# fujii-team/deComP

Measured on AMD Instinct MI355X. Metric: nmf_mu_iterations_per_s, higher is better.
Workload: dtype f32

## Files before the change

### decomp_amd/csrc/gemm.hpp

```cpp
#pragma once
#include <type_traits>

#include "gemm_generic.hpp"
#include "gemm_mfma_bf16x6.hpp"
#include "gemm_mfma_f32.hpp"
#include "gemm_mfma_f64.hpp"
#include "scalar.hpp"

namespace dcp {

enum GemmForm { FORM_NT = 0, FORM_NN = 1, FORM_TN = 2 };
enum TileSel { TILE_AUTO = 0, TILE_LARGE = 1, TILE_SMALL = 2, TILE_HUGE = 3, TILE_SMALL_DEEP = 4, TILE_MID = 5 };

template <class T>
struct GemmArgs {
    const T* A = nullptr;
    long lda = 0;
    const T* B = nullptr;
    long ldb = 0;
    const T* B2 = nullptr;
    long ldb2 = 0;
    int n_b1 = 0;
    const T* A2 = nullptr;
    long lda2 = 0;
// ... 316 lines not shown
    } else {
        if constexpr (std::is_same<T, c64>::value) {
            if (cplx_on_mfma<FORM>(a.conjA, a.conjB, a.ext_ws)) {
                GemmProblem p;
                const float* Ar = reinterpret_cast<const float*>(a.A);
                p.A = Ar; p.lda = 2 * a.lda;
                p.B2 = nullptr; p.ldb2 = 0; p.n_b1 = 2 * a.N;
                p.ksplits = a.ksplits; p.klen = a.klen;
                p.tiles_m = p.tiles_n = 0;
                p.mt_fast = (FORM == FORM_NT) ? 0 : 1;
                constexpr int AL = (FORM == FORM_TN) ? XMAJOR : KMAJOR;
                constexpr int BL = (FORM == FORM_NT) ? KMAJOR : XMAJOR;
                if constexpr (FORM == FORM_TN) {
                    p.B = reinterpret_cast<const float*>(a.B); p.ldb = 2 * a.ldb;
                    if (a.B2 != nullptr) {
                        p.B2 = reinterpret_cast<const float*>(a.B2); p.ldb2 = 2 * a.ldb2;
                        p.n_b1 = 2 * a.n_b1;
                    }
                    p.M = 2 * a.M; p.N = 2 * a.N; p.K = a.K;
                    CplxTnEpi<Epi> ce{epi};
                    const int tier = pick_tier<FORM>(p.M, p.N, p.K, a.tile, a.split_planned);
                    if (tier == TIER_SMALL || tier == TIER_SMALL_DEEP || tier == TIER_FLAT || tier == TIER_TALL)
                        return launch_gemm_mfma<CfgSmall, AL, BL>(stream, p, ce);
                    if (!tn_plain_schedule()) return launch_gemm_mfma<CfgLargeX, AL, BL>(stream, p, ce);
                    return launch_gemm_mfma<CfgLarge, AL, BL>(stream, p, ce);
                } else if (cplx_planar_a<FORM>(a.M, a.N, a.conjA, a.conjB, a.ext_ws)) {
                    if (a.A_rows != nullptr) {
                        p.A = a.A_rows; p.lda = a.lda_rows;
                    } else {
                        long g = ((long)a.M * a.K + 255) / 256;
                        if (g > 4096) g = 4096;
                        if (g < 1) g = 1;
                        hipLaunchKernelGGL((cplx_rows_kernel<float>), dim3((unsigned)g), dim3(256), 0, stream, a.A,
                                           (long)a.M, (long)a.K, a.lda, a.ext_ws);
                        p.A = a.ext_ws; p.lda = a.K;
                    }
                    p.B = reinterpret_cast<const float*>(a.B); p.ldb = 2 * a.ldb;
                    p.M = 2 * a.M; p.N = 2 * a.N; p.K = a.K;
                    if (a.ksplits <= 1) p.klen = 0;
                    CplxNnEpi<Epi> ce{epi};
                    const int tier = pick_tier<FORM>(p.M, p.N, p.K, a.tile, a.split_planned);
                    if (tier == TIER_SMALL_DEEP) return launch_gemm_mfma<CfgSmallDeep, AL, BL>(stream, p, ce);
                    if (tier == TIER_SMALL || tier == TIER_FLAT || tier == TIER_TALL)
                        return launch_gemm_mfma<CfgSmall, AL, BL>(stream, p, ce);
                    return launch_gemm_mfma<CfgLarge, AL, BL>(stream, p, ce);
                } else {
                    const long rowsB = (FORM == FORM_NT) ? a.N : a.K;
                    const long colsB = (FORM == FORM_NT) ? a.K : a.N;
                    long g = (rowsB * colsB + 255) / 256;
                    if (g > 4096) g = 4096;
                    if (g < 1) g = 1;
                    if (!a.ext_ready)
                        hipLaunchKernelGGL((cplx_ext_kernel<float>), dim3((unsigned)g), dim3(256), 0, stream, a.B,
                                           rowsB, colsB, a.ldb, a.ext_ws);
                    p.B = a.ext_ws; p.ldb = 2 * colsB;
                    p.M = a.M; p.N = 2 * a.N; p.K = 2 * a.K;
                    if (a.ksplits <= 1) p.klen = 0;
                    CplxColEpi<Epi> ce{epi};
                    const int tier = pick_tier<FORM>(p.M, p.N, p.K, a.tile, a.split_planned);
                    if (tier == TIER_SMALL || tier == TIER_SMALL_DEEP || tier == TIER_FLAT || tier == TIER_TALL)
                        return launch_gemm_mfma<CfgSmall, AL, BL>(stream, p, ce);
                    if (tier == TIER_HUGE) return launch_gemm_mfma<CfgHuge, AL, BL>(stream, p, ce);
                    if (tier == TIER_MID) return launch_gemm_mfma<CfgMid, AL, BL>(stream, p, ce);
                    return launch_gemm_mfma<CfgLarge, AL, BL>(stream, p, ce);
                }
            }
        }
        if constexpr (std::is_same<T, c128>::value) {
            const int Me = (FORM == FORM_TN) ? 2 * a.M : a.M;
            const int t128 = f64_tier(Me, 2 * a.N, a.tile);
            if (cplx_on_mfma<FORM>(a.conjA, a.conjB, a.ext_ws) && t128 != F64_GENERIC) {
                GemmProblemD p;
                p.A = reinterpret_cast<const double*>(a.A); p.lda = 2 * a.lda;
                p.B2 = nullptr; p.ldb2 = 0; p.n_b1 = 2 * a.N;
                p.ksplits = a.ksplits; p.klen = a.klen;
                p.tiles_m = p.tiles_n = 0;
                p.mt_fast = (FORM == FORM_NT) ? 0 : 1;
                constexpr int AL = (FORM == FORM_TN) ? XMAJOR : KMAJOR;
                constexpr int BL = (FORM == FORM_NT) ? KMAJOR : XMAJOR;
                if constexpr (FORM == FORM_TN) {
                    p.B = reinterpret_cast<const double*>(a.B); p.ldb = 2 * a.ldb;
                    if (a.B2 != nullptr) {
                        p.B2 = reinterpret_cast<const double*>(a.B2); p.ldb2 = 2 * a.ldb2;
                        p.n_b1 = 2 * a.n_b1;
                    }
                    p.M = 2 * a.M; p.N = 2 * a.N; p.K = a.K;
                    CplxTnEpi<Epi, double> ce{epi};
                    return launch_f64_tier<AL, BL>(t128, stream, p, ce);
                } else if (cplx_planar_a<FORM>(a.M, a.N, a.conjA, a.conjB, a.ext_ws) &&
                           f64_tier(2 * a.M, 2 * a.N, a.tile) != F64_GENERIC) {
                    if (a.A_rows != nullptr) {
                        p.A = a.A_rows; p.lda = a.lda_rows;
                    } else {
                        long g = ((long)a.M * a.K + 255) / 256;
                        if (g > 4096) g = 4096;
                        if (g < 1) g = 1;
                        hipLaunchKernelGGL((cplx_rows_kernel<double>), dim3((unsigned)g), dim3(256), 0, stream, a.A,
                                           (long)a.M, (long)a.K, a.lda, a.ext_ws);
                        p.A = a.ext_ws; p.lda = a.K;
                    }
                    p.B = reinterpret_cast<const double*>(a.B); p.ldb = 2 * a.ldb;
                    p.M = 2 * a.M; p.N = 2 * a.N; p.K = a.K;
                    if (a.ksplits <= 1) p.klen = 0;
                    CplxNnEpi<Epi, double> ce{epi};
                    return launch_f64_tier<AL, BL>(f64_tier(p.M, p.N, a.tile), stream, p, ce);
                } else {
                    const long rowsB = (FORM == FORM_NT) ? a.N : a.K;
                    const long colsB = (FORM == FORM_NT) ? a.K : a.N;
                    long g = (rowsB * colsB + 255) / 256;
                    if (g > 4096) g = 4096;
                    if (g < 1) g = 1;
                    if (!a.ext_ready)
                        hipLaunchKernelGGL((cplx_ext_kernel<double>), dim3((unsigned)g), dim3(256), 0, stream, a.B,
                                           rowsB, colsB, a.ldb, a.ext_ws);
                    p.B = a.ext_ws; p.ldb = 2 * colsB;
                    p.M = a.M; p.N = 2 * a.N; p.K = 2 * a.K;
                    if (a.ksplits <= 1) p.klen = 0;
                    CplxColEpi<Epi, double> ce{epi};
                    return launch_f64_tier<AL, BL>(t128, stream, p, ce);
                }
            }
        }
        if constexpr (std::is_same<T, double>::value) {
            const int t64 = f64_tier(a.M, a.N, a.tile, a.K);
            if (t64 != F64_GENERIC) {
                GemmProblemD p;
                p.A = a.A; p.lda = a.lda; p.B = a.B; p.ldb = a.ldb;
                p.B2 = a.B2; p.ldb2 = a.ldb2; p.n_b1 = a.n_b1;
                p.M = a.M; p.N = a.N; p.K = a.K;
                p.ksplits = a.ksplits; p.klen = a.klen;
                p.tiles_m = p.tiles_n = 0;
                p.mt_fast = (FORM == FORM_NT) ? 0 : 1;
                constexpr int AL = (FORM == FORM_TN) ? XMAJOR : KMAJOR;
                constexpr int BL = (FORM == FORM_NT) ? KMAJOR : XMAJOR;
                return launch_f64_tier<AL, BL>(t64, stream, p, epi);
            }
        }
        GenericProblem<T> p;
        p.A = a.A; p.B = a.B; p.B2 = a.B2; p.n_b1 = a.n_b1;
        if (FORM == FORM_TN) { p.sAm = 1; p.sAk = a.lda; } else { p.sAm = a.lda; p.sAk = 1; }
        if (FORM == FORM_NT) { p.sBk = 1; p.sBn = a.ldb; p.sB2k = 1; p.sB2n = a.ldb2; }
        else { p.sBk = a.ldb; p.sBn = 1; p.sB2k = a.ldb2; p.sB2n = 1; }
        p.M = a.M; p.N = a.N; p.K = a.K;
        p.ksplits = a.ksplits; p.klen = a.klen;
        p.tiles_m = p.tiles_n = 0;
        if constexpr (scalar_traits<T>::is_complex)
            return launch_gemm_generic<T, Epi>(stream, p, a.conjA, a.conjB, epi);
        else
            return launch_gemm_generic<T, Epi>(stream, p, false, false, epi);
    }
}

enum { X6_NONE = -1, X6_LARGE = 0, X6_HUGE = 1 };

template <int FORM>
inline GemmProblem x6_problem(const GemmArgs<float>& a) {
    GemmProblem p;
    p.A = a.A; p.lda = a.lda; p.B = a.B; p.ldb = a.ldb;
    p.B2 = a.B2; p.ldb2 = a.ldb2; p.n_b1 = a.n_b1;
    p.A2 = a.A2; p.lda2 = a.lda2; p.m_a1 = a.m_a1;
    p.M = a.M; p.N = a.N; p.K = a.K;
    p.ksplits = a.ksplits; p.klen = a.klen;
    p.tiles_m = p.tiles_n = 0;
    p.mt_fast = (FORM == FORM_NT) ? 0 : 1;
    return p;
}

template <int FORM>
inline int x6_tier(const GemmArgs<float>& a) {
    if (FORM == FORM_NN) return X6_NONE;
    const int tier = pick_tier<FORM>(a.M, a.N, a.K, a.tile, a.split_planned, true);
    const GemmProblem p = x6_problem<FORM>(a);
    if (FORM == FORM_NT && tier == TIER_HUGE && x6_eligible<X6Huge>(p)) return X6_HUGE;
    if ((tier == TIER_LARGE || (FORM == FORM_NT && (tier == TIER_MID || tier == TIER_HUGE))) &&
        x6_eligible<X6Large>(p))
        return X6_LARGE;
    return X6_NONE;
}

template <int FORM, class Epi>
inline hipError_t gemm_bf16x6(hipStream_t stream, const GemmArgs<float>& a, const Epi& epi) {
    constexpr int AL = (FORM == FORM_TN) ? XMAJOR : KMAJOR;
    constexpr int BL = (FORM == FORM_NT) ? KMAJOR : XMAJOR;
    if constexpr (FORM == FORM_NN) {
        return hipErrorInvalidValue;
    } else {
        const int t = x6_tier<FORM>(a);
        if (t == X6_HUGE) return launch_gemm_bf16x6<X6Huge, AL, BL, Epi>(stream, x6_problem<FORM>(a), epi);
        if (t == X6_LARGE) return launch_gemm_bf16x6<X6Large, AL, BL, Epi>(stream, x6_problem<FORM>(a), epi);
        return hipErrorInvalidValue;
    }
}


inline bool al16_ptr(const void* q) { return (reinterpret_cast<uintptr_t>(q) & 15) == 0; }

template <class T>
struct EpiStore {
    static constexpr bool kVec4 = false;
    T* C;
    long ldc;
    __device__ __forceinline__ void operator()(int r, int c, T v, int) const {
        C[(long)r * ldc + c] = v;
    }
    bool vec_ok() const { return al16_ptr(C) && (ldc % 4) == 0; }
    __device__ __forceinline__ void vec4(int r, int c0, f32x4 v, int) const {
        *reinterpret_cast<f32x4*>(reinterpret_cast<float*>(C) + (long)r * ldc + c0) = v;
    }
};

template <class T>
struct EpiSlab {
    static constexpr bool kVec4 = false;
    T* slab;
    long ldc;
    long slab_stride;
    __device__ __forceinline__ void operator()(int r, int c, T v, int s) const {
        slab[(long)s * slab_stride + (long)r * ldc + c] = v;
    }
    bool vec_ok() const { return al16_ptr(slab) && (ldc % 4) == 0 && (slab_stride % 4) == 0; }
    __device__ __forceinline__ void vec4(int r, int c0, f32x4 v, int s) const {
        *reinterpret_cast<f32x4*>(reinterpret_cast<float*>(slab) + (long)s * slab_stride + (long)r * ldc + c0) = v;
    }
    static constexpr bool kVec2 = std::is_same<T, float>::value;
    bool vec2_ok() const {
        return (reinterpret_cast<uintptr_t>(slab) & 7) == 0 && (ldc % 2) == 0 && (slab_stride % 2) == 0;
    }
    __device__ __forceinline__ void store2(int r, int c0, float v0, float v1, int s) const {
        typedef float f32x2 __attribute__((ext_vector_type(2)));
        *reinterpret_cast<f32x2*>(reinterpret_cast<float*>(slab) + (long)s * slab_stride + (long)r * ldc + c0) =
            f32x2{v0, v1};
    }
};

template <class T>
struct EpiMuNum {
    static constexpr bool kVec4 = std::is_same<T, float>::value;
    const T* cur;
    long ld_cur;
    const T* den;
    long ld_den;
    T* out;
    long ld_out;
    __device__ __forceinline__ void operator()(int r, int c, T v, int) const {
        const T d = den[(long)r * ld_den + c];
        out[(long)r * ld_out + c] = cur[(long)r * ld_cur + c] * max_np(v, T(0)) /
                                    max_np(d, T(1.0e-15));
    }
    bool vec_ok() const {
        return al16_ptr(cur) && al16_ptr(den) && al16_ptr(out) && (ld_cur % 4) == 0 && (ld_den % 4) == 0 &&
               (ld_out % 4) == 0;
    }
    __device__ __forceinline__ void vec4(int r, int c0, f32x4 v, int) const {
        const f32x4 d = *reinterpret_cast<const f32x4*>(reinterpret_cast<const float*>(den) + (long)r * ld_den + c0);
        const f32x4 x = *reinterpret_cast<const f32x4*>(reinterpret_cast<const float*>(cur) + (long)r * ld_cur + c0);
        f32x4 o;
#pragma unroll
        for (int e = 0; e < 4; ++e) o[e] = x[e] * max_np(v[e], 0.0f) / max_np(d[e], 1.0e-15f);
        *reinterpret_cast<f32x4*>(reinterpret_cast<float*>(out) + (long)r * ld_out + c0) = o;
    }
};

template <class T>
struct EpiMuDen {
    const T* cur;
    long ld_cur;
    const T* num;
    long ld_num;
    T* out;
    long ld_out;
    __device__ __forceinline__ void operator()(int r, int c, T v, int) const {
        const T nu = num[(long)r * ld_num + c];
        out[(long)r * ld_out + c] = cur[(long)r * ld_cur + c] * max_np(nu, T(0)) /
                                    max_np(v, T(1.0e-15));
    }
};

template <class T>
struct EpiMuDenSlabs {
    static constexpr bool kVec4 = std::is_same<T, float>::value;
    const T* cur;
    long ld_cur;
    const T* slabs;
    long ld_slab;
    long slab_stride;
    int S;
    T* out;
    long ld_out;
    __device__ __forceinline__ void operator()(int r, int c, T v, int) const {
        const long o = (long)r * ld_slab + c;
        T nu = slabs[o];
        for (int s = 1; s < S; ++s) nu = nu + slabs[(long)s * slab_stride + o];
        out[(long)r * ld_out + c] = cur[(long)r * ld_cur + c] * max_np(nu, T(0)) / max_np(v, T(1.0e-15));
    }
    bool vec_ok() const {
        return al16_ptr(cur) && al16_ptr(slabs) && al16_ptr(out) && (ld_cur % 4) == 0 && (ld_slab % 4) == 0 &&
               (slab_stride % 4) == 0 && (ld_out % 4) == 0;
    }
    __device__ __forceinline__ void vec4(int r, int c0, f32x4 v, int) const {
        if constexpr (std::is_same<T, float>::value) {
            const long o = (long)r * ld_slab + c0;
            f32x4 nu = *reinterpret_cast<const f32x4*>(slabs + o);
            for (int s = 1; s < S; ++s) {
                const f32x4 p = *reinterpret_cast<const f32x4*>(slabs + (long)s * slab_stride + o);
#pragma unroll
                for (int e = 0; e < 4; ++e) nu[e] = nu[e] + p[e];
            }
            const f32x4 x = *reinterpret_cast<const f32x4*>(cur + (long)r * ld_cur + c0);
            f32x4 q;
#pragma unroll
            for (int e = 0; e < 4; ++e) q[e] = x[e] * max_np(nu[e], 0.0f) / max_np(v[e], 1.0e-15f);
            *reinterpret_cast<f32x4*>(out + (long)r * ld_out + c0) = q;
        }
    }
};

template <class T>
struct EpiMulMask {
    const real_t<T>* mask;
    long ld_mask;
    T* out;
    long ld_out;
    __device__ __forceinline__ void operator()(int r, int c, T v, int) const {
        out[(long)r * ld_out + c] = scale(v, mask[(long)r * ld_mask + c]);
    }
    static constexpr bool kVec4 = std::is_same<T, float>::value;
// ... 78 lines not shown
```

### decomp_amd/csrc/gemm_mfma_bf16x6.hpp

```cpp
#pragma once
#include "gemm_mfma_f32.hpp"

namespace dcp {

typedef __bf16 x6_bf16x4 __attribute__((ext_vector_type(4)));
typedef __bf16 x6_bf16x8 __attribute__((ext_vector_type(8)));

template <int BM_, int BN_, int WM_, int WN_, int MINW_>
struct X6Cfg {
    static constexpr int BM = BM_, BN = BN_, BK = 16, WM = WM_, WN = WN_, MINW = MINW_;
    static constexpr int NWAVES = (BM_ / WM_) * (BN_ / WN_);
    static constexpr int NTHREADS = 64 * NWAVES;
};
typedef X6Cfg<256, 256, 64, 64, 1> X6Huge;
typedef X6Cfg<128, 128, 64, 64, 2> X6Large;

template <int ROWS>
struct X6Panel {
    static constexpr int PLANE_BYTES = ROWS * 32;
    static constexpr int BYTES = 3 * PLANE_BYTES;
};

__device__ __forceinline__ int x6_chunk(int r, int q) { return r * 32 + ((q ^ ((r >> 3) & 1)) << 4); }

__device__ __forceinline__ void x6_split(f32x4 a, x6_bf16x4& h, x6_bf16x4& m, x6_bf16x4& l) {
    h = __builtin_convertvector(a, x6_bf16x4);
    const f32x4 r1 = a - __builtin_convertvector(h, f32x4);
    m = __builtin_convertvector(r1, x6_bf16x4);
    const f32x4 r2 = r1 - __builtin_convertvector(m, f32x4);
    l = __builtin_convertvector(r2, x6_bf16x4);
}

template <int LAY, int ROWS, int NT, int G>
__device__ __forceinline__ void x6_gload(f32x4 (&r)[G], const float* __restrict__ p, long ld, int row0, int k0,
                                         int tid) {
    static_assert(G * NT * 4 == ROWS * 16, "panel must be a whole number of 4-k groups per thread");
#pragma unroll
    for (int i = 0; i < G; ++i) {
        const int idx = tid + i * NT;
        if (LAY == KMAJOR) {
            const int row = idx >> 2, kq = idx & 3;
            r[i] = *reinterpret_cast<const f32x4*>(p + (long)(row0 + row) * ld + (k0 + 4 * kq));
        } else {
            const int row = idx % ROWS, kq = idx / ROWS;
            const float* q = p + (long)(k0 + 4 * kq) * ld + (row0 + row);
#pragma unroll
            for (int e = 0; e < 4; ++e) r[i][e] = q[(long)e * ld];
        }
    }
}

template <int LAY, int ROWS, int NT, int G>
__device__ __forceinline__ void x6_lds_store(char* s, const f32x4 (&r)[G], int tid) {
#pragma unroll
    for (int i = 0; i < G; ++i) {
        const int idx = tid + i * NT;
        int row, kq;
        if (LAY == KMAJOR) { row = idx >> 2; kq = idx & 3; }
        else { row = idx % ROWS; kq = idx / ROWS; }
        const int off = x6_chunk(row, kq >> 1) + ((kq & 1) << 3);
        x6_bf16x4 h, m, l;
        x6_split(r[i], h, m, l);
        *reinterpret_cast<x6_bf16x4*>(s + off) = h;
        *reinterpret_cast<x6_bf16x4*>(s + X6Panel<ROWS>::PLANE_BYTES + off) = m;
        *reinterpret_cast<x6_bf16x4*>(s + 2 * X6Panel<ROWS>::PLANE_BYTES + off) = l;
    }
}

template <class Cfg, int ALAY, int BLAY, class Epi>
__global__ void __launch_bounds__(Cfg::NTHREADS, Cfg::MINW) gemm_bf16x6_kernel(GemmProblem p, Epi epi) {
    constexpr int BM = Cfg::BM, BN = Cfg::BN, BK = Cfg::BK, WM = Cfg::WM, WN = Cfg::WN;
    constexpr int TM = WM / 32, TN = WN / 32;
    constexpr int WAVES_N = BN / WN;
    constexpr int NT = Cfg::NTHREADS;
    constexpr int GA = BM * BK / 4 / NT, GB = BN * BK / 4 / NT;
    constexpr int PA = X6Panel<BM>::PLANE_BYTES, PB = X6Panel<BN>::PLANE_BYTES;
    constexpr int BUF = X6Panel<BM>::BYTES + X6Panel<BN>::BYTES;
    static_assert(epi_mode<Epi>::value == 0 && !epi_rowbits<Epi>::value, "bf16x6 core: plain real epilogues");

    extern __shared__ __attribute__((aligned(16))) char x6_smem[];

    const int tid = threadIdx.x;
    const int lane = tid & 63, wave = tid >> 6;
    const int wm = wave / WAVES_N, wn = wave % WAVES_N;
    const int l31 = lane & 31, h = lane >> 5;

    const int lid = xcd_remap(blockIdx.x, gridDim.x);
    const int tiles = p.tiles_m * p.tiles_n;
    const int split = lid / tiles;
    const int t = lid - split * tiles;
    int mt, nt;
    if (p.mt_fast) {
        mt = t % p.tiles_m;
        nt = t / p.tiles_m;
    } else {
        nt = t % p.tiles_n;
        mt = t / p.tiles_n;
    }
    const int m0 = mt * BM;
    const int kbeg = split * p.klen;
    const int kend = min(p.K, kbeg + p.klen);
    const float* Bp = p.B;
    long ldb = p.ldb;
    int nB0 = nt * BN;
    int n0 = nB0;
    if (nt >= p.tiles_n1) {
        Bp = p.B2;
        ldb = p.ldb2;
        nB0 = (nt - p.tiles_n1) * BN;
        n0 = p.n_b1 + nB0;
    }

    f32x16 acc[TM][TN];
#pragma unroll
    for (int i = 0; i < TM; ++i)
#pragma unroll
        for (int j = 0; j < TN; ++j)
#pragma unroll
            for (int r = 0; r < 16; ++r) acc[i][j][r] = 0.0f;

    f32x4 ra[GA], rb[GB];
    const int nkb = (kend - kbeg) / BK;
    if (nkb > 0) {
        x6_gload<ALAY, BM, NT>(ra, p.A, p.lda, m0, kbeg, tid);
        x6_gload<BLAY, BN, NT>(rb, Bp, ldb, nB0, kbeg, tid);
        x6_lds_store<ALAY, BM, NT>(x6_smem, ra, tid);
        x6_lds_store<BLAY, BN, NT>(x6_smem + X6Panel<BM>::BYTES, rb, tid);
    }
    __syncthreads();

    int aoff[TM], boff[TN];
#pragma unroll
    for (int i = 0; i < TM; ++i) aoff[i] = x6_chunk(wm * WM + i * 32 + l31, h);
#pragma unroll
    for (int j = 0; j < TN; ++j) boff[j] = x6_chunk(wn * WN + j * 32 + l31, h);

    for (int kb = 0; kb < nkb; ++kb) {
        const int cur = kb & 1;
        const char* sA = x6_smem + cur * BUF;
        const char* sB = sA + X6Panel<BM>::BYTES;
        const bool more = (kb + 1) < nkb;
        if (more) {
            const int k0 = kbeg + (kb + 1) * BK;
            x6_gload<ALAY, BM, NT>(ra, p.A, p.lda, m0, k0, tid);
            x6_gload<BLAY, BN, NT>(rb, Bp, ldb, nB0, k0, tid);
        }
        x6_bf16x8 fb[3][TN];
#pragma unroll
        for (int pl = 0; pl < 3; ++pl)
#pragma unroll
            for (int j = 0; j < TN; ++j) fb[pl][j] = *reinterpret_cast<const x6_bf16x8*>(sB + pl * PB + boff[j]);
        constexpr int TA[6] = {2, 0, 1, 1, 0, 0};
        constexpr int TB[6] = {0, 2, 1, 0, 1, 0};
#pragma unroll
        for (int i = 0; i < TM; ++i) {
            x6_bf16x8 fa[3];
#pragma unroll
            for (int pl = 0; pl < 3; ++pl) fa[pl] = *reinterpret_cast<const x6_bf16x8*>(sA + pl * PA + aoff[i]);
#pragma unroll
            for (int tt = 0; tt < 6; ++tt)
#pragma unroll
                for (int j = 0; j < TN; ++j)
                    acc[i][j] = __builtin_amdgcn_mfma_f32_32x32x16_bf16(fa[TA[tt]], fb[TB[tt]][j], acc[i][j], 0, 0, 0);
            __builtin_amdgcn_sched_barrier(0);
        }
        if (more) {
            char* nxt = x6_smem + (cur ^ 1) * BUF;
            x6_lds_store<ALAY, BM, NT>(nxt, ra, tid);
            x6_lds_store<BLAY, BN, NT>(nxt + X6Panel<BM>::BYTES, rb, tid);
        }
        __syncthreads();
    }

    if constexpr (epi_vec4<Epi>::value) {
        const int tq = l31 & 3, col0 = (l31 & ~3);
#pragma unroll
        for (int i = 0; i < TM; ++i)
#pragma unroll
            for (int j = 0; j < TN; ++j)
#pragma unroll
                for (int g = 0; g < 4; ++g) {
                    f32x4 x;
#pragma unroll
                    for (int e = 0; e < 4; ++e) x[e] = acc[i][j][4 * g + e];
                    const f32x4 y = quad_transpose(x, tq);
                    epi.vec4(m0 + wm * WM + i * 32 + 8 * g + 4 * h + tq, n0 + wn * WN + j * 32 + col0, y, split);
                }
    } else {
#pragma unroll
        for (int i = 0; i < TM; ++i)
#pragma unroll
            for (int j = 0; j < TN; ++j) {
                const int col = n0 + wn * WN + j * 32 + l31;
#pragma unroll
                for (int r = 0; r < 16; ++r) {
                    const int row = m0 + wm * WM + i * 32 + (r & 3) + 8 * (r >> 2) + 4 * h;
                    epi(row, col, acc[i][j][r], split);
                }
            }
    }
}

template <class Epi>
inline bool x6_epi_ok(const Epi& epi) {
    if constexpr (epi_vec4<Epi>::value) return epi.vec_ok();
    else return true;
}

template <class Cfg>
inline bool x6_eligible(const GemmProblem& p) {
    auto al16 = [](const void* q) { return (reinterpret_cast<uintptr_t>(q) & 15) == 0; };
    const int n1 = p.B2 != nullptr ? p.n_b1 : p.N;
    bool ok = p.M > 0 && p.N > 0 && p.K > 0 && (p.M % Cfg::BM) == 0 && (n1 % Cfg::BN) == 0 &&
              ((p.N - n1) % Cfg::BN) == 0 && (p.K % 16) == 0 && p.A2 == nullptr && (p.lda % 4) == 0 &&
              (p.ldb % 4) == 0 && al16(p.A) && al16(p.B);
    if (p.B2 != nullptr) ok = ok && (p.ldb2 % 4) == 0 && al16(p.B2);
    if (p.ksplits > 1) ok = ok && (p.klen % 16) == 0 && p.klen > 0;
    return ok;
}

template <class Cfg, int ALAY, int BLAY, class Epi>
inline hipError_t launch_gemm_bf16x6(hipStream_t stream, GemmProblem p, const Epi& epi) {
    if (!x6_eligible<Cfg>(p) || !x6_epi_ok(epi)) return hipErrorInvalidValue;
    if (p.B2 == nullptr) p.n_b1 = p.N;
    p.m_a1 = p.M;
    p.tiles_m1 = p.tiles_m = p.M / Cfg::BM;
    p.tiles_n1 = p.n_b1 / Cfg::BN;
    p.tiles_n = p.tiles_n1 + (p.N - p.n_b1) / Cfg::BN;
    if (p.ksplits < 1) p.ksplits = 1;
    if (p.ksplits == 1) p.klen = p.K;
    p.vec_epi = epi_vec4<Epi>::value ? 1 : 0;
    p.al_mask = 0;
    const int grid = p.tiles_m * p.tiles_n * p.ksplits;
    if (grid <= 0) return hipSuccess;
    constexpr int lds_bytes = 2 * (X6Panel<Cfg::BM>::BYTES + X6Panel<Cfg::BN>::BYTES);
    const void* fn = reinterpret_cast<const void*>(&gemm_bf16x6_kernel<Cfg, ALAY, BLAY, Epi>);
    if constexpr (lds_bytes > 65536) {
        static DynLdsRaised raised;
        std::atomic<bool>& done = raised.on_current_device();
        if (!done) {
            hipError_t e = hipFuncSetAttribute(fn, hipFuncAttributeMaxDynamicSharedMemorySize, lds_bytes);
            if (e != hipSuccess) return e;
            done = true;
        }
    }
    hipLaunchKernelGGL((gemm_bf16x6_kernel<Cfg, ALAY, BLAY, Epi>), dim3(grid), dim3(Cfg::NTHREADS), lds_bytes,
                       stream, p, epi);
    return hipGetLastError();
}

}
```

### decomp_amd/csrc/nmf_impl.hpp

```cpp
#pragma once
#include <math.h>

#include "gemm.hpp"
#include "handle.hpp"
#include "kernels_small.hpp"

namespace dcp {

inline int64_t nmf_stats_width(int64_t F, int64_t K, int likelihood, bool masked) {
    return (likelihood == DCP_LIK_L2 && !masked) ? (F + K) : 2 * F;
}

constexpr int kSplitTarget = 1024;
constexpr int kMaxSplits = 64;

template <class T>
struct NmfShape {
    int64_t N, F, K;
    int lik;
    bool masked;
};

template <class T>
struct NmfStatsWs {
    T* Q = nullptr;
    T* G = nullptr;
    T* f = nullptr;
    T* Ym = nullptr;
    T* slabs = nullptr;
    T* vecK = nullptr;
    T* part = nullptr;
    size_t slab_count = 0;
    const uint32_t* mbits = nullptr;
};

template <class T>
inline int nmf_xupdate_splits(int64_t N, int64_t F, int64_t K, GemmArgs<T>& pg) {
    pg.M = (int)N; pg.N = (int)K; pg.K = (int)F;
    pg.tile = TILE_AUTO;
    int bm = 64, bn = 64;
    if (std::is_same<T, float>::value) tier_dims(pick_tier<FORM_NT>(pg.M, pg.N, pg.K, TILE_AUTO, true), bm, bn);
    const long tiles = (long)ceil_div(N, bm) * ceil_div(K, bn);
    const long enough = (bm == 256) ? 192 : 512;
    if (tiles >= enough || F < 1024) {
        pg.ksplits = 1;
        return 1;
    }
    plan_splits<FORM_NT>(pg, (bm == 256) ? 256 : 1024, 8);
    return pg.ksplits;
}

template <class T>
inline size_t nmf_slab_elems(const NmfShape<T>& s) {
    const int64_t W = nmf_stats_width(s.F, s.K, s.lik, s.masked);
    GemmArgs<T> a;
    a.M = (int)s.K; a.N = (int)W; a.K = (int)s.N;
    plan_splits<FORM_TN>(a, kSplitTarget, kMaxSplits);
    size_t stats_slabs = (size_t)a.ksplits * s.K * W;
    GemmArgs<T> g;
    g.M = (int)s.K; g.N = (int)s.K; g.K = (int)s.F;
    plan_splits<FORM_NT>(g, 512, kMaxSplits, 16);
    size_t g_slabs = (size_t)g.ksplits * s.K * s.K;
    GemmArgs<T> pg;
    const int ps = nmf_xupdate_splits<T>(s.N, s.F, s.K, pg);
    size_t x_slabs = ps > 1 ? (size_t)ps * s.N * s.K : 0;
    if (ps > 1 && s.masked && s.lik == DCP_LIK_L2) {
        GemmArgs<T> sg;
        const int ss = nmf_xupdate_splits<T>(2 * s.N, s.F, s.K, sg);
        const size_t st_slabs = (size_t)(ss > 1 ? ss : 1) * 2 * s.N * s.K;
        if (st_slabs > x_slabs) x_slabs = st_slabs;
    }
    size_t m = stats_slabs > g_slabs ? stats_slabs : g_slabs;
    return m > x_slabs ? m : x_slabs;
}

template <class T>
inline void nmf_plan_stats(WsPlan& plan, const NmfShape<T>& s, bool need_ym) {
    const bool gram = (s.lik == DCP_LIK_L2 && !s.masked);
    plan.add<T>((size_t)s.N * s.K);
    if (gram) plan.add<T>((size_t)s.K * s.K);
    if (!gram) plan.add<T>((size_t)s.N * s.F);
    if (need_ym) plan.add<T>((size_t)s.N * s.F);
    plan.add<T>(nmf_slab_elems(s));
    plan.add<T>((size_t)s.K);
    plan.add<T>((size_t)64 * (s.K > s.F ? s.K : s.F));
}

template <class T>
inline int nmf_carve_stats(dcp_handle* h, NmfStatsWs<T>& w, const NmfShape<T>& s, bool need_ym) {
    const bool gram = (s.lik == DCP_LIK_L2 && !s.masked);
    w.Q = ws_alloc<T>(h, (size_t)s.N * s.K);
    if (gram) w.G = ws_alloc<T>(h, (size_t)s.K * s.K);
    if (!gram) w.f = ws_alloc<T>(h, (size_t)s.N * s.F);
    if (need_ym) w.Ym = ws_alloc<T>(h, (size_t)s.N * s.F);
    w.slab_count = nmf_slab_elems(s);
    w.slabs = ws_alloc<T>(h, w.slab_count);
    w.vecK = ws_alloc<T>(h, (size_t)s.K);
    w.part = ws_alloc<T>(h, (size_t)64 * (s.K > s.F ? s.K : s.F));
    if (!w.Q || !w.slabs || !w.vecK || !w.part || (gram && !w.G) || (!gram && !w.f) ||
        (need_ym && !w.Ym))
        return fail(h, DCP_ERR_INTERNAL, "nmf workspace plan mismatch");
    return DCP_OK;
}

template <class T>
struct NmfUpdateWs {
    T* U = nullptr;
    T* rowmax = nullptr;
};
template <class T>
inline void nmf_plan_update(WsPlan& plan, int64_t F, int64_t K) {
    plan.add<T>((size_t)K * F);
    plan.add<T>((size_t)K);
}
template <class T>
inline int nmf_carve_update(dcp_handle* h, NmfUpdateWs<T>& w, int64_t F, int64_t K) {
    w.U = ws_alloc<T>(h, (size_t)K * F);
    w.rowmax = ws_alloc<T>(h, (size_t)K);
    if (!w.U || !w.rowmax) return fail(h, DCP_ERR_INTERNAL, "nmf workspace plan mismatch");
    return DCP_OK;
}

#define DCP_LAUNCH_OK(h, what)                                                        \
    do {                                                                              \
        hipError_t _e = (what);                                                       \
        if (_e != hipSuccess)                                                         \
            return dcp::fail((h), DCP_ERR_HIP, std::string("launch failed: ") +       \
                                                   hipGetErrorString(_e));            \
    } while (0)

template <class T>
inline int column_sums(dcp_handle* h, const T* a, long ld, long rows, long cols, T* part, T* out) {
    const int stripes = rows >= 64 ? 64 : (rows > 0 ? (int)rows : 1);
    const long rows_per = (rows + stripes - 1) / stripes;
    dim3 grid(grid_for(cols, 64), stripes);
    hipLaunchKernelGGL((colsum_partial_kernel<T>), grid, dim3(256), 0, h->stream, a, ld, rows,
                       cols, rows_per, part);
    DCP_LAUNCH_OK(h, hipGetLastError());
    hipLaunchKernelGGL((reduce_slabs_kernel<T>), dim3(grid_for(cols, 64)), dim3(256), 0, h->stream,
                       part, cols, stripes, cols, out);
    DCP_LAUNCH_OK(h, hipGetLastError());
    return DCP_OK;
}

template <int FORM, class T, class Epi>
inline hipError_t nmf_product(dcp_handle* h, hipStream_t st, const GemmArgs<T>& a, const Epi& epi, bool split_ok) {
    if constexpr (std::is_same<T, float>::value) {
        if (split_ok && h->f32_product_mode == 0 && x6_tier<FORM>(a) != X6_NONE && x6_epi_ok(epi))
            return gemm_bf16x6<FORM>(st, a, epi);
    }
    return gemm<FORM>(st, a, epi);
}

template <class T>
inline int nmf_stats(dcp_handle* h, const T* Ypre, const T* mask, const T* Xin, T* Xout, const T* D,
                     const NmfShape<T>& s, T* stats, NmfStatsWs<T>& w, int phases = 3) {
    hipStream_t st = h->stream;
    const int N = (int)s.N, F = (int)s.F, K = (int)s.K;
    const bool gram = (s.lik == DCP_LIK_L2 && !s.masked);
    const int W = (int)nmf_stats_width(s.F, s.K, s.lik, s.masked);

    auto forward = [&](const T* X) -> int {
        ProfScope ps(h, DCP_PROF_FWD);
        GemmArgs<T> fa;
        fa.A = X; fa.lda = K; fa.B = D; fa.ldb = F; fa.M = N; fa.N = F; fa.K = K;
        if (s.lik == DCP_LIK_L2) {
            if constexpr (std::is_same<T, float>::value) {
                if (w.mbits != nullptr) {
                    DCP_LAUNCH_OK(h, (gemm<FORM_NN>(st, fa, EpiMulMaskBits{w.mbits, (long)F, w.f, (long)F})));
                    return DCP_OK;
                }
            }
            DCP_LAUNCH_OK(h, (gemm<FORM_NN>(st, fa, EpiMulMask<T>{mask, F, w.f, F})));
        } else
            DCP_LAUNCH_OK(h, (gemm<FORM_NN>(st, fa, EpiKlRatio<T>{Ypre, F, nullptr, 0, w.f, F})));
        return DCP_OK;
    };

    const T* X = Xin;
    bool x_done = false;
    if (phases & 1) {
    const T* xnum_A = Ypre;
    const T* xden = w.Q;
    long ld_xden = K;
    GemmArgs<T> pg_probe;
    const bool split_gram = gram && std::is_same<T, float>::value && Xout != Xin &&
                            nmf_xupdate_splits<T>(s.N, s.F, s.K, pg_probe) > 1;
    if (gram) {
        {
            ProfScope ps(h, DCP_PROF_GRAM);
            GemmArgs<T> g;
            g.A = D; g.lda = F; g.B = D; g.ldb = F; g.M = K; g.N = K; g.K = F;
            if (!std::is_same<T, float>::value) g.tile = TILE_SMALL_DEEP;
            plan_splits<FORM_NT>(g, 512, kMaxSplits, 16);
            DCP_LAUNCH_OK(h, (gemm<FORM_NT>(st, g, EpiSlab<T>{w.slabs, K, (long)K * K})));
            hipLaunchKernelGGL((reduce_slabs_kernel<T>), dim3(grid_for((long)K * K)), dim3(256), 0,
                               st, w.slabs, (long)K * K, g.ksplits, (long)K * K, w.G);
            DCP_LAUNCH_OK(h, hipGetLastError());
        }
        if (!split_gram) {
            ProfScope ps(h, DCP_PROF_XNEG);
            GemmArgs<T> q;
            q.A = Xin; q.lda = K; q.B = w.G; q.ldb = K; q.M = N; q.N = K; q.K = K;
            DCP_LAUNCH_OK(h, (gemm<FORM_NN>(st, q, EpiStore<T>{w.Q, K})));
        }
    } else if (s.lik == DCP_LIK_L2) {
        DCP_TRY(forward(Xin));
        if constexpr (std::is_same<T, float>::value) {
            GemmArgs<T> sg;
            sg.A = w.f; sg.lda = F; sg.A2 = Ypre; sg.lda2 = F; sg.m_a1 = N;
            sg.B = D; sg.ldb = F; sg.M = 2 * N; sg.N = K; sg.K = F;
            GemmArgs<T> probe;
            const bool split_single = nmf_xupdate_splits<T>(s.N, s.F, s.K, probe) > 1;
            if (split_single && (N % 256) == 0 && (F % 16) == 0) {
                ProfScope ps(h, DCP_PROF_XUPDATE);
                nmf_xupdate_splits<T>(2 * s.N, s.F, s.K, sg);
                sg.A = w.f; sg.lda = F; sg.A2 = Ypre; sg.lda2 = F; sg.m_a1 = N;
                sg.B = D; sg.ldb = F;
                if (sg.ksplits < 1) sg.ksplits = 1;
                if ((size_t)sg.ksplits * 2 * N * K > w.slab_count)
                    return fail(h, DCP_ERR_INTERNAL, "nmf stacked x-update slab plan mismatch");
                DCP_LAUNCH_OK(h, (gemm<FORM_NT>(st, sg, EpiSlab<T>{w.slabs, K, (long)2 * N * K})));
                hipLaunchKernelGGL((mu_quotient_stacked_kernel<T>), dim3(grid_for((long)N * K)), dim3(256), 0,
                                   st, Xin, (const T*)w.slabs, (long)2 * N * K, sg.ksplits, (long)N * K, Xout);
                DCP_LAUNCH_OK(h, hipGetLastError());
                x_done = true;
            }
        }
        if (!x_done) {
            ProfScope ps(h, DCP_PROF_XNEG);
            GemmArgs<T> q;
            q.A = w.f; q.lda = F; q.B = D; q.ldb = F; q.M = N; q.N = K; q.K = F;
            DCP_LAUNCH_OK(h, (gemm<FORM_NT>(st, q, EpiStore<T>{w.Q, K})));
        }
    } else {
        DCP_TRY(forward(Xin));
        xnum_A = w.f;
        ProfScope ps(h, DCP_PROF_XNEG);
        if (!s.masked) {
            hipLaunchKernelGGL((rowsum_kernel<T>), dim3(K), dim3(256), 0, st, D, (long)F, (long)F,
                               w.vecK);
            DCP_LAUNCH_OK(h, hipGetLastError());
            xden = w.vecK;
            ld_xden = 0;
        } else {
            GemmArgs<T> q;
            q.A = mask; q.lda = F; q.B = D; q.ldb = F; q.M = N; q.N = K; q.K = F;
            DCP_LAUNCH_OK(h, (gemm<FORM_NT>(st, q, EpiStore<T>{w.Q, K})));
        }
    }
    if (!x_done) {
        ProfScope ps(h, DCP_PROF_XUPDATE);
        GemmArgs<T> pg;
        pg.A = xnum_A; pg.lda = F; pg.B = D; pg.ldb = F; pg.M = N; pg.N = K; pg.K = F;
        const int psplits = nmf_xupdate_splits<T>(s.N, s.F, s.K, pg);
        if (psplits <= 1) {
            pg.ksplits = 1;
            DCP_LAUNCH_OK(h, (nmf_product<FORM_NT>(h, st, pg, EpiMuNum<T>{Xin, K, xden, ld_xden, Xout, K}, gram)));
        } else {
            if ((size_t)pg.ksplits * N * K > w.slab_count)
                return fail(h, DCP_ERR_INTERNAL, "nmf x-update slab plan mismatch");
            DCP_LAUNCH_OK(h, (nmf_product<FORM_NT>(h, st, pg, EpiSlab<T>{w.slabs, K, (long)N * K}, gram)));
            if (split_gram) {
                GemmArgs<T> q;
                q.A = Xin; q.lda = K; q.B = w.G; q.ldb = K; q.M = N; q.N = K; q.K = K;
                DCP_LAUNCH_OK(h, (gemm<FORM_NN>(st, q, EpiMuDenSlabs<T>{Xin, K, w.slabs, K, (long)N * K,
                                                                        pg.ksplits, Xout, K})));
            } else {
                hipLaunchKernelGGL((mu_quotient_slabs_kernel<T>), dim3(grid_for((long)N * K)), dim3(256),
                                   0, st, Xin, (const T*)w.slabs, (long)N * K, pg.ksplits, xden,
                                   (long)ld_xden, (long)N, (long)K, Xout);
                DCP_LAUNCH_OK(h, hipGetLastError());
            }
        }
    }
    X = Xout;
    }
    if (!(phases & 2)) return DCP_OK;

    GemmArgs<T> sa;
    sa.A = X; sa.lda = K; sa.M = K; sa.N = W; sa.K = N;
    if (gram) {
        sa.B = Ypre; sa.ldb = F; sa.B2 = X; sa.ldb2 = K; sa.n_b1 = F;
    } else if (s.lik == DCP_LIK_L2) {
        DCP_TRY(forward(X));
        sa.B = Ypre; sa.ldb = F; sa.B2 = w.f; sa.ldb2 = F; sa.n_b1 = F;
    } else {
        DCP_TRY(forward(X));
        if (s.masked) {
            sa.B = w.f; sa.ldb = F; sa.B2 = mask; sa.ldb2 = F; sa.n_b1 = F;
        } else {
            sa.B = w.f; sa.ldb = F; sa.N = F;
        }
    }
    const int Wg = sa.N;
    plan_splits<FORM_TN>(sa, kSplitTarget, kMaxSplits);
    if ((size_t)sa.ksplits * K * Wg > w.slab_count)
        return fail(h, DCP_ERR_INTERNAL, "nmf slab plan mismatch");
    {
        ProfScope ps(h, DCP_PROF_STATS);
        DCP_LAUNCH_OK(h, (nmf_product<FORM_TN>(h, st, sa, EpiSlab<T>{w.slabs, Wg, (long)K * Wg}, gram)));
    }
    ProfScope ps(h, DCP_PROF_STATS_SUM);
    if (Wg == W) {
        launch_reduce_slabs<T>(st, w.slabs, (long)K * W, sa.ksplits, (long)K * W, stats);
        DCP_LAUNCH_OK(h, hipGetLastError());
    } else {
        hipLaunchKernelGGL((reduce_slabs_rows_kernel<T>), dim3(grid_for((long)K * F)), dim3(256), 0,
                           st, w.slabs, (long)K * F, sa.ksplits, (long)K, (long)F, stats, (long)W);
        DCP_LAUNCH_OK(h, hipGetLastError());
        DCP_TRY(column_sums<T>(h, X, K, N, K, w.part, w.vecK));
        hipLaunchKernelGGL((bcast_rows_kernel<T>), dim3(grid_for((long)K * F)), dim3(256), 0, st,
                           w.vecK, (long)K, (long)F, stats + F, (long)W);
        DCP_LAUNCH_OK(h, hipGetLastError());
    }
    return DCP_OK;
}

template <class T>
inline int nmf_grad_x(dcp_handle* h, const T* Ypre, const T* mask, const T* X, const T* D,
                      const NmfShape<T>& s, T* pos, T* neg, NmfStatsWs<T>& w) {
    hipStream_t st = h->stream;
    const int N = (int)s.N, F = (int)s.F, K = (int)s.K;
    const bool gram = (s.lik == DCP_LIK_L2 && !s.masked);
    const T* pos_A = Ypre;
    if (gram) {
        GemmArgs<T> g;
        g.A = D; g.lda = F; g.B = D; g.ldb = F; g.M = K; g.N = K; g.K = F;
        plan_splits<FORM_NT>(g, 512, kMaxSplits, 16);
        DCP_LAUNCH_OK(h, (gemm<FORM_NT>(st, g, EpiSlab<T>{w.slabs, K, (long)K * K})));
        hipLaunchKernelGGL((reduce_slabs_kernel<T>), dim3(grid_for((long)K * K)), dim3(256), 0, st, w.slabs,
                           (long)K * K, g.ksplits, (long)K * K, w.G);
        DCP_LAUNCH_OK(h, hipGetLastError());
        GemmArgs<T> q;
        q.A = X; q.lda = K; q.B = w.G; q.ldb = K; q.M = N; q.N = K; q.K = K;
        DCP_LAUNCH_OK(h, (gemm<FORM_NN>(st, q, EpiStore<T>{neg, K})));
    } else {
        GemmArgs<T> fa;
        fa.A = X; fa.lda = K; fa.B = D; fa.ldb = F; fa.M = N; fa.N = F; fa.K = K;
        if (s.lik == DCP_LIK_L2) {
            DCP_LAUNCH_OK(h, (gemm<FORM_NN>(st, fa, EpiMulMask<T>{mask, F, w.f, F})));
            GemmArgs<T> q;
            q.A = w.f; q.lda = F; q.B = D; q.ldb = F; q.M = N; q.N = K; q.K = F;
            DCP_LAUNCH_OK(h, (gemm<FORM_NT>(st, q, EpiStore<T>{neg, K})));
        } else {
            DCP_LAUNCH_OK(h, (gemm<FORM_NN>(st, fa, EpiKlRatio<T>{Ypre, F, nullptr, 0, w.f, F})));
            pos_A = w.f;
            if (!s.masked) {
                hipLaunchKernelGGL((rowsum_kernel<T>), dim3(K), dim3(256), 0, st, D, (long)F, (long)F, w.vecK);
                DCP_LAUNCH_OK(h, hipGetLastError());
                hipLaunchKernelGGL((bcast_cols_kernel<T>), dim3(grid_for((long)N * K)), dim3(256), 0, st,
                                   (const T*)w.vecK, (long)N, (long)K, neg);
                DCP_LAUNCH_OK(h, hipGetLastError());
            } else {
                GemmArgs<T> q;
                q.A = mask; q.lda = F; q.B = D; q.ldb = F; q.M = N; q.N = K; q.K = F;
                DCP_LAUNCH_OK(h, (gemm<FORM_NT>(st, q, EpiStore<T>{neg, K})));
            }
        }
    }
    GemmArgs<T> pg;
    pg.A = pos_A; pg.lda = F; pg.B = D; pg.ldb = F; pg.M = N; pg.N = K; pg.K = F;
    DCP_LAUNCH_OK(h, (gemm<FORM_NT>(st, pg, EpiStore<T>{pos, K})));
    return DCP_OK;
}

template <class T>
inline int nmf_update(dcp_handle* h, const T* stats, const T* D, T* D_new, int64_t F64, int64_t K64,
                      int lik, bool masked, T* maxdiff_dev, NmfUpdateWs<T>& w,
                      T* maxdiff_next = nullptr, unsigned int* ticket = nullptr, T* host_out = nullptr) {
    hipStream_t st = h->stream;
    const int F = (int)F64, K = (int)K64;
    const bool gram = (lik == DCP_LIK_L2 && !masked);
    const int W = (int)nmf_stats_width(F64, K64, lik, masked);
    {
        ProfScope ps(h, DCP_PROF_DUPDATE);
        if (gram) {
            GemmArgs<T> a;
            a.A = stats + F; a.lda = W; a.B = D; a.ldb = F; a.M = K; a.N = F; a.K = K;
            if (std::is_same<T, float>::value) a.tile = (K % 64 == 0) ? TILE_SMALL_DEEP : TILE_SMALL;
            else a.tile = TILE_AUTO;
            DCP_LAUNCH_OK(h, (gemm<FORM_NN>(st, a, EpiMuDen<T>{D, F, stats, W, w.U, F})));
        } else {
            hipLaunchKernelGGL((mu_quotient_kernel<T>), dim3(grid_for((long)K * F)), dim3(256), 0,
                               st, D, (long)F, stats, (long)W, stats + F, (long)W, 0, (long)K,
                               (long)F, w.U, (long)F);
            DCP_LAUNCH_OK(h, hipGetLastError());
        }
    }
    ProfScope ps(h, DCP_PROF_DNORM);
    if (maxdiff_next != nullptr) {
        hipLaunchKernelGGL((row_normalize_kernel<T>), dim3(K), dim3(256), 0, st, w.U, (long)F,
                           (long)F, 1, D, (long)F, D_new, (long)F, (T*)nullptr, (T*)nullptr,
                           maxdiff_dev, maxdiff_next, ticket, host_out);
        DCP_LAUNCH_OK(h, hipGetLastError());
        return DCP_OK;
    }
    hipLaunchKernelGGL((row_normalize_kernel<T>), dim3(K), dim3(256), 0, st, w.U, (long)F, (long)F,
                       1, D, (long)F, D_new, (long)F, w.rowmax, (T*)nullptr, (T*)nullptr,
                       (T*)nullptr);
    DCP_LAUNCH_OK(h, hipGetLastError());
    hipLaunchKernelGGL((final_max_kernel<T>), dim3(1), dim3(256), 0, st, w.rowmax, (long)K,
                       maxdiff_dev);
    DCP_LAUNCH_OK(h, hipGetLastError());
    return DCP_OK;
}

template <class T>
inline int nmf_residual(dcp_handle* h, const T* Y, const T* mask, const T* X, const T* D, int64_t N,
                        int64_t F, int64_t K, T* tmpNF, double* partial_dev, int nblocks) {
    GemmArgs<T> a;
    a.A = X; a.lda = K; a.B = D; a.ldb = F; a.M = (int)N; a.N = (int)F; a.K = (int)K;
    DCP_LAUNCH_OK(h, (gemm<FORM_NN>(h->stream, a, EpiResidual<T>{Y, F, mask, F, tmpNF, F})));
    hipLaunchKernelGGL((sumsq_partial_kernel<T>), dim3(nblocks), dim3(256), 0, h->stream, tmpNF,
                       (long)N * F, partial_dev);
    DCP_LAUNCH_OK(h, hipGetLastError());
    return DCP_OK;
}

}

namespace dcp {

template <class T>
inline int nmf_mask_prepare(dcp_handle* h, const T* Y, const T* mask, int64_t N, int64_t F, T* Ym,
                            uint32_t* bits, int* flag_dev, int* binary) {
    hipLaunchKernelGGL((mul_mask_kernel<T>), dim3(grid_for(N * F)), dim3(256), 0, h->stream, Y, mask,
                       (long)N, (long)F, (long)F, Ym);
    DCP_LAUNCH_OK(h, hipGetLastError());
    *binary = 0;
    if (!std::is_same<T, float>::value || bits == nullptr) return DCP_OK;
    void* hostv = nullptr;
    DCP_TRY(host_scratch(h, 64, &hostv));
    DCP_HIP_OK(h, hipMemsetAsync(flag_dev, 0, sizeof(int), h->stream));
    hipLaunchKernelGGL((mask_rowbits_kernel<T>), dim3(grid_for(((N + 31) / 32) * F)), dim3(256), 0,
                       h->stream, mask, (long)N, (long)F, bits, flag_dev);
    DCP_LAUNCH_OK(h, hipGetLastError());
    DCP_HIP_OK(h, hipMemcpyAsync(hostv, flag_dev, sizeof(int), hipMemcpyDeviceToHost, h->stream));
    DCP_HIP_OK(h, hipStreamSynchronize(h->stream));
    *binary = (*reinterpret_cast<int*>(hostv) == 0) ? 1 : 0;
    return DCP_OK;
}

inline size_t mask_bits_words(int64_t N, int64_t F) { return (size_t)((N + 31) / 32) * (size_t)F; }

}
```

Before: 604.8.

## Route NMF stats TN GEMM to huge bf16x6 tile with transposed LDS reads

Lets the f32 TN stats product in the Gram path use the 256x256 bf16x6 kernel, with its own split-K plan targeting about 256 tile-splits, and reserves enough slab workspace for it. The X-major global load becomes a vectorized f32x4 load along rows. Fragments now come from a new XOR-swizzled LDS layout read with ds_read_tr16 transpose instructions, replacing four strided scalar loads per group. The aim is to cut global load count and per-tile overhead for the stats GEMM, at the cost of fewer workgroups, more shared memory per block, and an extra split plan to keep consistent with slab sizing.

Result: faster. 673.9, median of 6 (+11.4%).

```diff
diff --git a/decomp_amd/csrc/gemm.hpp b/decomp_amd/csrc/gemm.hpp
--- a/decomp_amd/csrc/gemm.hpp
+++ b/decomp_amd/csrc/gemm.hpp
@@ -492,6 +492,7 @@
 }
 
 enum { X6_NONE = -1, X6_LARGE = 0, X6_HUGE = 1 };
+constexpr int kX6HugeTnMinK = 1024;
 
 template <int FORM>
 inline GemmProblem x6_problem(const GemmArgs<float>& a) {
@@ -506,12 +507,42 @@
     return p;
 }
 
+template <class T>
+inline bool x6_huge_tn_shape(const GemmArgs<T>& a, int n1, int klen) {
+    return std::is_same<T, float>::value && a.A2 == nullptr && a.M > 0 && a.N > 0 && a.K > 0 &&
+           a.M % X6Huge::BM == 0 && n1 % X6Huge::BN == 0 && (a.N - n1) % X6Huge::BN == 0 && klen >= kX6HugeTnMinK &&
+           pick_tier<FORM_TN>(a.M, a.N, a.K, a.tile, true, true) == TIER_LARGE;
+}
+
+template <class T>
+inline bool plan_splits_x6_tn(GemmArgs<T>& a, int n1, int max_splits) {
+    if (a.M <= 0 || a.N <= 0 || a.K <= 0 || a.M % X6Huge::BM || n1 % X6Huge::BN || (a.N - n1) % X6Huge::BN)
+        return false;
+    const long tiles = (long)(a.M / X6Huge::BM) * (n1 / X6Huge::BN + (a.N - n1) / X6Huge::BN);
+    const long kblocks = ceil_div(a.K, 16);
+    long smax = kblocks / 32;
+    if (smax < 1) smax = 1;
+    if (smax > max_splits) smax = max_splits;
+    long s = 256 / tiles;
+    if (s > smax) s = smax;
+    if (s < 1) s = 1;
+    const int klen = (int)(((kblocks + s - 1) / s) * 16);
+    if (!x6_huge_tn_shape(a, n1, klen)) return false;
+    a.split_planned = true;
+    a.klen = klen;
+    a.ksplits = ceil_div(a.K, klen);
+    return true;
+}
+
 template <int FORM>
 inline int x6_tier(const GemmArgs<float>& a) {
     if (FORM == FORM_NN) return X6_NONE;
     const int tier = pick_tier<FORM>(a.M, a.N, a.K, a.tile, a.split_planned, true);
     const GemmProblem p = x6_problem<FORM>(a);
     if (FORM == FORM_NT && tier == TIER_HUGE && x6_eligible<X6Huge>(p)) return X6_HUGE;
+    if (FORM == FORM_TN && tier == TIER_LARGE && x6_huge_tn_shape(a, a.B2 != nullptr ? a.n_b1 : a.N, a.ksplits > 1 ? a.klen : a.K) &&
+        x6_eligible<X6Huge>(p))
+        return X6_HUGE;
     if ((tier == TIER_LARGE || (FORM == FORM_NT && (tier == TIER_MID || tier == TIER_HUGE))) &&
         x6_eligible<X6Large>(p))
         return X6_LARGE;
diff --git a/decomp_amd/csrc/gemm_mfma_bf16x6.hpp b/decomp_amd/csrc/gemm_mfma_bf16x6.hpp
--- a/decomp_amd/csrc/gemm_mfma_bf16x6.hpp
+++ b/decomp_amd/csrc/gemm_mfma_bf16x6.hpp
@@ -34,7 +34,7 @@
 template <int LAY, int ROWS, int NT, int G>
 __device__ __forceinline__ void x6_gload(f32x4 (&r)[G], const float* __restrict__ p, long ld, int row0, int k0,
                                          int tid) {
-    static_assert(G * NT * 4 == ROWS * 16, "panel must be a whole number of 4-k groups per thread");
+    static_assert(G * NT * 4 == ROWS * 16, "panel must be a whole number of 4-value groups per thread");
 #pragma unroll
     for (int i = 0; i < G; ++i) {
         const int idx = tid + i * NT;
@@ -42,12 +42,16 @@
             const int row = idx >> 2, kq = idx & 3;
             r[i] = *reinterpret_cast<const f32x4*>(p + (long)(row0 + row) * ld + (k0 + 4 * kq));
         } else {
-            const int row = idx % ROWS, kq = idx / ROWS;
-            const float* q = p + (long)(k0 + 4 * kq) * ld + (row0 + row);
-#pragma unroll
-            for (int e = 0; e < 4; ++e) r[i][e] = q[(long)e * ld];
-        }
-    }
+            const int g = idx % (ROWS / 4), k = idx / (ROWS / 4);
+            r[i] = *reinterpret_cast<const f32x4*>(p + (long)(k0 + k) * ld + (row0 + 4 * g));
+        }
+    }
+}
+
+template <int ROWS>
+__device__ __forceinline__ int x6_granule(int k, int g) {
+    static_assert(ROWS >= 128, "the XOR swizzle needs 32 granules per k row");
+    return k * (ROWS * 2) + ((g ^ ((k & 3) << 3)) << 3);
 }
 
 template <int LAY, int ROWS, int NT, int G>
@@ -55,16 +59,37 @@
 #pragma unroll
     for (int i = 0; i < G; ++i) {
         const int idx = tid + i * NT;
-        int row, kq;
-        if (LAY == KMAJOR) { row = idx >> 2; kq = idx & 3; }
-        else { row = idx % ROWS; kq = idx / ROWS; }
-        const int off = x6_chunk(row, kq >> 1) + ((kq & 1) << 3);
+        int off;
+        if (LAY == KMAJOR) {
+            const int row = idx >> 2, kq = idx & 3;
+            off = x6_chunk(row, kq >> 1) + ((kq & 1) << 3);
+        } else {
+            off = x6_granule<ROWS>(idx / (ROWS / 4), idx % (ROWS / 4));
+        }
         x6_bf16x4 h, m, l;
         x6_split(r[i], h, m, l);
         *reinterpret_cast<x6_bf16x4*>(s + off) = h;
         *reinterpret_cast<x6_bf16x4*>(s + X6Panel<ROWS>::PLANE_BYTES + off) = m;
         *reinterpret_cast<x6_bf16x4*>(s + 2 * X6Panel<ROWS>::PLANE_BYTES + off) = l;
     }
+}
+
+template <int LAY, int ROWS>
+__device__ __forceinline__ int x6_frag_off(int r0, int lane) {
+    const int l31 = lane & 31, h = lane >> 5;
+    if (LAY == KMAJOR) return x6_chunk(r0 + l31, h);
+    const int q = (lane >> 2) & 3, pq = lane & 3, gh = (lane >> 4) & 1;
+    return x6_granule<ROWS>(8 * h + q, (r0 >> 2) + 4 * gh + pq);
+}
+
+template <int LAY, int ROWS>
+__device__ __forceinline__ x6_bf16x8 x6_frag(const char* plane, int off) {
+    if (LAY == KMAJOR) return *reinterpret_cast<const x6_bf16x8*>(plane + off);
+    typedef short s16x4 __attribute__((ext_vector_type(4)));
+    typedef __attribute__((address_space(3))) s16x4 lds_s16x4;
+    const s16x4 lo = __builtin_amdgcn_ds_read_tr16_b64_v4i16((lds_s16x4*)(plane + off));
+    const s16x4 hi = __builtin_amdgcn_ds_read_tr16_b64_v4i16((lds_s16x4*)(plane + off + 4 * ROWS * 2));
+    return __builtin_bit_cast(x6_bf16x8, __builtin_shufflevector(lo, hi, 0, 1, 2, 3, 4, 5, 6, 7));
 }
 
 template <class Cfg, int ALAY, int BLAY, class Epi>
@@ -131,9 +156,9 @@
 
     int aoff[TM], boff[TN];
 #pragma unroll
-    for (int i = 0; i < TM; ++i) aoff[i] = x6_chunk(wm * WM + i * 32 + l31, h);
-#pragma unroll
-    for (int j = 0; j < TN; ++j) boff[j] = x6_chunk(wn * WN + j * 32 + l31, h);
+    for (int i = 0; i < TM; ++i) aoff[i] = x6_frag_off<ALAY, BM>(wm * WM + i * 32, lane);
+#pragma unroll
+    for (int j = 0; j < TN; ++j) boff[j] = x6_frag_off<BLAY, BN>(wn * WN + j * 32, lane);
 
     for (int kb = 0; kb < nkb; ++kb) {
         const int cur = kb & 1;
@@ -149,14 +174,14 @@
 #pragma unroll
         for (int pl = 0; pl < 3; ++pl)
 #pragma unroll
-            for (int j = 0; j < TN; ++j) fb[pl][j] = *reinterpret_cast<const x6_bf16x8*>(sB + pl * PB + boff[j]);
+            for (int j = 0; j < TN; ++j) fb[pl][j] = x6_frag<BLAY, BN>(sB + pl * PB, boff[j]);
         constexpr int TA[6] = {2, 0, 1, 1, 0, 0};
         constexpr int TB[6] = {0, 2, 1, 0, 1, 0};
 #pragma unroll
         for (int i = 0; i < TM; ++i) {
             x6_bf16x8 fa[3];
 #pragma unroll
-            for (int pl = 0; pl < 3; ++pl) fa[pl] = *reinterpret_cast<const x6_bf16x8*>(sA + pl * PA + aoff[i]);
+            for (int pl = 0; pl < 3; ++pl) fa[pl] = x6_frag<ALAY, BM>(sA + pl * PA, aoff[i]);
 #pragma unroll
             for (int tt = 0; tt < 6; ++tt)
 #pragma unroll
diff --git a/decomp_amd/csrc/nmf_impl.hpp b/decomp_amd/csrc/nmf_impl.hpp
--- a/decomp_amd/csrc/nmf_impl.hpp
+++ b/decomp_amd/csrc/nmf_impl.hpp
@@ -57,6 +57,12 @@
     a.M = (int)s.K; a.N = (int)W; a.K = (int)s.N;
     plan_splits<FORM_TN>(a, kSplitTarget, kMaxSplits);
     size_t stats_slabs = (size_t)a.ksplits * s.K * W;
+    if (s.lik == DCP_LIK_L2 && !s.masked) {
+        GemmArgs<T> b;
+        b.M = (int)s.K; b.N = (int)W; b.K = (int)s.N;
+        if (plan_splits_x6_tn(b, (int)s.F, kMaxSplits) && (size_t)b.ksplits * s.K * W > stats_slabs)
+            stats_slabs = (size_t)b.ksplits * s.K * W;
+    }
     GemmArgs<T> g;
     g.M = (int)s.K; g.N = (int)s.K; g.K = (int)s.F;
     plan_splits<FORM_NT>(g, 512, kMaxSplits, 16);
@@ -294,7 +300,9 @@
         }
     }
     const int Wg = sa.N;
-    plan_splits<FORM_TN>(sa, kSplitTarget, kMaxSplits);
+    const bool x6_allowed = std::is_same<T, float>::value && h->f32_product_mode == 0;
+    if (!(gram && x6_allowed && plan_splits_x6_tn(sa, sa.n_b1, kMaxSplits)))
+        plan_splits<FORM_TN>(sa, kSplitTarget, kMaxSplits);
     if ((size_t)sa.ksplits * K * Wg > w.slab_count)
         return fail(h, DCP_ERR_INTERNAL, "nmf slab plan mismatch");
     {
```
